# yanqinJiang/Animate3D

Hardware: AMD Instinct MI355X
Metric: UNet denoise-steps/sec, 4view×16frame×512² MV-VDM @1/2/4/8 GPU (higher is better)
Workload: dtype bf16; 1 GPU; BASELINE config 2: 4 views x 16 frames x 512^2 px (64x64 latent), CFG-doubled batch V=8 videos, one MVUNetMotionModel.forward per step, SD1.5 MV-VDM UNet 1.53 B params, seeded synthetic weights; parallelism=single GPU

## Files before the change

animate3d_amd/csrc/gemm_common.h:

```cpp
#pragma once
#include "common.h"

struct GemmParams {
  const uint16_t* X; int64_t ldx;
  const uint16_t* W; int64_t ldw;
  const float* bias;
  const uint16_t* rowbias; int64_t rb_div;
  const uint16_t* R; int64_t ldr;
  uint16_t* Y; int64_t ldy;
  int64_t M, N, K;
  float alpha, beta;
  int vec16;
  int out_f32;
  int B, H, Wd, Cin, Ho, Wo, stride, up, He, We;
  int64_t tiles_n, tiles_m;
  int ksplit, nk_item;
  float* ws; int64_t ws_bytes;
  const uint16_t* X2; int64_t ldx2; int64_t K1;
};

constexpr int EPI_LINEAR = 0, EPI_GEGLU = 1;

static inline int a3d_gemm_kernel_of(int flags) { return flags & A3D_GEMM_KERNEL_MASK; }
static inline int a3d_gemm_reserved_cus_of(int flags) { return flags & A3D_GEMM_RESERVED_CUS_MASK; }
// ... 106 lines not shown
  }
}

template <int NB> A3D_DEV void read_frags(const char* stage, uint32_t xrd, uint32_t wrd, uint32_t wrd_last, uint32_t ko, u32x4_t (&fx)[2],
                                          u32x4_t (&fw)[NB]) {
  const char* xs = stage + xrd;
  const char* ws = stage + wrd;
  const char* wl = stage + wrd_last;
#pragma unroll
  for (int tm = 0; tm < 2; ++tm) fx[tm] = *reinterpret_cast<const u32x4_t*>(xs + tm * 4096 + ko);
#pragma unroll
  for (int tn = 0; tn < NB - 1; ++tn) fw[tn] = *reinterpret_cast<const u32x4_t*>(ws + tn * 4096 + ko);
  fw[NB - 1] = *reinterpret_cast<const u32x4_t*>(wl + ko);
}

template <int EPI, int NB>
A3D_DEV void epilogue_rounded(const GemmParams& p, f32x16_t (&acc)[NB][2], float* const stg, const float* const bias_lds,
                              const uint16_t* const rowbias_lds, const int64_t m0, const int64_t n0, const int wm, const WaveCols<NB> wc,
                              const int lane) {
  const int wblk = wc.first, wblk_last = wc.last;
  auto pass_cols = [&](int ps) { return (2 * ps + 1 < NB) ? 64 : 32; };
  auto pass_col0 = [&](int ps) { return ((2 * ps + 1 < NB) ? wblk + 2 * ps : wblk_last) * 32; };
  const int l31 = lane & 31, g = lane >> 5;
  constexpr int NP = (NB + 1) / 2;
  constexpr int RS = (EPI == EPI_GEGLU) ? 64 : 128;
  char* const stg16 = reinterpret_cast<char*>(stg);
  const int wsw = (EPI == EPI_GEGLU) ? ((l31 >> 1) & 3) : (l31 & 7);
  const int whalf = 8 * (g ^ ((l31 >> 3) & 1));
  auto unswap = [](u32x4_t o, int row) {
    const bool sw = row & 8;
    u32x4_t r;
    r[0] = sw ? o[2] : o[0]; r[1] = sw ? o[3] : o[1]; r[2] = sw ? o[0] : o[2]; r[3] = sw ? o[1] : o[3];
    return r;
  };
// ... 96 lines not shown
      else quads(std::false_type{});
      wave_lds_fence();
      const int lpr = ncol / 8;
      const int cc = lane & (lpr - 1);
      u32x4_t ob[4];
#pragma unroll
      for (int j = 0; j < 4; ++j) {
        if (j * (64 / lpr) >= 32) continue;
        const int row = (64 / lpr) * j + lane / lpr;
        ob[j] = *reinterpret_cast<const u32x4_t*>(sb + row * RS + 16 * (cc ^ (row & 7)));
      }
#pragma unroll
      for (int j = 0; j < 4; ++j) {
        if (j * (64 / lpr) >= 32) continue;
        const int row = (64 / lpr) * j + lane / lpr;
        const int64_t m = mbase + row;
        const u32x4_t o = unswap(ob[j], row);
        *reinterpret_cast<u32x4_t*>(p.Y + m * p.ldy + nbase + 8 * cc) = o;
      }
    }
  }
}

template <int NB>
A3D_DEV void epilogue_residual(const GemmParams& p, f32x16_t (&acc)[NB][2], float* const stg, const float* const bias_lds,
                               const uint16_t* const rowbias_lds, const int64_t m0, const int64_t n0, const int wm, const WaveCols<NB> wc,
                               const int lane) {
  const int l31 = lane & 31, g = lane >> 5;
  constexpr int SROW = 68;
  constexpr int NP = WaveCols<NB>::PASSES;
  u32x4_t rres[2][4];
// ... 78 lines not shown
```

animate3d_amd/csrc/gemm_conv.hip:

```cpp
#include "gemm_common.h"

namespace {

constexpr int BM = 128, BN = 128;
template <int BKT> struct TileCfg {
  static constexpr int LROW = BKT + 8;
  static constexpr int TILE_ELEMS = 128 * LROW;
  static constexpr int STAGE_BYTES = 2 * 2 * TILE_ELEMS * 2;
  static constexpr int EPI_BYTES = 4 * 32 * 68 * 4;
  static constexpr int SMEM_BYTES = STAGE_BYTES > EPI_BYTES ? STAGE_BYTES : EPI_BYTES;
  static constexpr int CPR = BKT / 8;
  static constexpr int RPT = 256 / CPR;
  static constexpr int NPASS = 128 / RPT;
};



template <int CONV, int EPI, int BKT, bool RES>
__global__ __launch_bounds__(256, (BKT == 64 ? 2 : 3)) void gemm_kernel(const GemmParams p) {
  using TC = TileCfg<BKT>;
  constexpr int LROW = TC::LROW, TILE_ELEMS = TC::TILE_ELEMS, NPASS = TC::NPASS, RPT = TC::RPT, BK = BKT;
  extern __shared__ __attribute__((aligned(16))) uint16_t smem[];
  const int tid = threadIdx.x;
  const int lane = tid & 63, wid = tid >> 6;
// ... 537 lines not shown
}

extern "C" int A3D_FN(a3d_conv3x3)(a3d_stream_t stream, const void* X, const void* Wp, const float* bias,
                                const void* rowbias, int64_t rb_div, const void* R, void* Y,
                                int B, int H, int W, int Cin, int Cout, int stride, int up2x, int flags) {
  return conv_entry(stream, X, Wp, bias, rowbias, rb_div, R, Y, B, H, W, Cin, Cout, stride, up2x, flags, nullptr, 0, nullptr);
}

extern "C" int A3D_FN(a3d_conv3x3_ws)(a3d_stream_t stream, const void* X, const void* Wp, const float* bias,
                                   const void* rowbias, int64_t rb_div, const void* R, void* Y,
                                   int B, int H, int W, int Cin, int Cout, int stride, int up2x, int flags,
                                   void* ws, int64_t ws_bytes, int64_t* ws_needed) {
  return conv_entry(stream, X, Wp, bias, rowbias, rb_div, R, Y, B, H, W, Cin, Cout, stride, up2x, flags, ws, ws_bytes, ws_needed);
}

extern "C" int A3D_FN(a3d_gemm_geglu)(a3d_stream_t stream, const void* X, int64_t ldx, const void* W, int64_t ldw,
                                   const float* bias, void* Y, int64_t ldy, int64_t M, int64_t N2, int64_t K, int flags) {
  GemmParams p = dense_params(X, ldx, W, ldw, bias, nullptr, 1, nullptr, 0, Y, ldy, M, N2, K, 1.f, 0.f);
  if (!dense_args_ok(p, 16, 64, 8)) return A3D_EINVAL;
  return launch<0, EPI_GEGLU>((hipStream_t)stream, p, flags);
}
```

animate3d_amd/csrc/gemm_pp.hip:

```cpp
#include "gemm_common.h"

namespace {

constexpr int PBM = 256;
template <int NB> struct PPCfg {
  static constexpr int BN = NB * 64;
  static constexpr int XBYTES = PBM * 128;
  static constexpr int WBYTES = BN * 128;
  static constexpr int EPI_BYTES = 8 * 32 * 68 * 4;
  static constexpr int STAGE = (XBYTES + WBYTES) > EPI_BYTES ? (XBYTES + WBYTES) : EPI_BYTES;
  static constexpr int BIAS_OFF = 2 * STAGE;
  static constexpr int SMEM = BIAS_OFF + 2 * BIAS_IMG_STRIDE;
};

constexpr int PP_GM = 8;
A3D_DEV void pp_tile_coords(int64_t t, int64_t tiles_m, int64_t tiles_n, int64_t& tile_m, int64_t& tile_n) {
  const int64_t gsz = PP_GM * tiles_n;
  const int64_t blk = t / gsz;
  const int64_t first = blk * PP_GM;
  const int64_t gm = tiles_m - first < PP_GM ? tiles_m - first : PP_GM;
  const int64_t within = t - blk * gsz;
  tile_n = within / gm;
  tile_m = first + (within - tile_n * gm);
}

template <int CONV, int EPI, int NB, bool RES, bool SPLIT = false, bool TWO = false>
__global__ __launch_bounds__(512, 1) void gemm_pp_kernel(const GemmParams p) {
  static_assert(!TWO || CONV == 0, "the two-source A operand is a dense-GEMM feature");
  using PC = PPCfg<NB>;
  constexpr int PH = 1, NPH = 4;
  constexpr int NP = 4 + NB;
  extern __shared__ __attribute__((aligned(16))) uint16_t smem[];
  char* const smem_b = reinterpret_cast<char*>(smem);
  const int tid = threadIdx.x, lane = tid & 63;
  const int wid = __builtin_amdgcn_readfirstlane(tid >> 6);
  const int wm = wid >> 1, wn = wid & 1;
  const int grp = wid >> 2;
  const int l31 = lane & 31, g = lane >> 5;
  const int lr = lane >> 3, pos = lane & 7;
  const uint32_t lds0 = lds_addr(smem);

  const int S = SPLIT ? p.ksplit : 1;
  const int64_t ntiles = p.tiles_m * p.tiles_n * S;
  const int64_t G = gridDim.x;
  int64_t t = xcd_remap(blockIdx.x, G);
  if (t >= ntiles) return;
// ... 1 lines not shown

  const uint32_t koff0 = (uint32_t)((g ^ ((l31 >> 1) & 7)) << 4);
  const uint32_t xrd = (uint32_t)(wm * 64 + l31) * 128u;
  const WaveCols<NB> wc(wn);
  const uint32_t wrd = (uint32_t)PC::XBYTES + (uint32_t)(wc.first * 32 + l31) * 128u;
  const uint32_t wrd_last = (uint32_t)PC::XBYTES + (uint32_t)(wc.last * 32 + l31) * 128u;

  const uint32_t vx0 = (uint32_t)(lr * p.ldx * 2 + ((pos ^ (lr >> 1)) << 4));
  const uint32_t vw0 = (uint32_t)(lr * p.ldw * 2 + ((pos ^ (lr >> 1)) << 4));
  uint32_t aoff[CONV ? 4 : 1];
  uint32_t amask[CONV ? 2 : 1];
  uint32_t sok[CONV ? 2 : 1];
  const int64_t cbias = CONV ? ((int64_t)p.Wd + 1) * p.Cin : 0;
  int64_t ld_m0 = 0, ld_n0 = 0;
  int ld_par = 0;
  int ik0 = 0, itap = 0, ikx = 0, iky = 0;
  uint64_t xck = 0;
  uint64_t zpage = 0;
  if constexpr (CONV != 0) {
    zpage = (uint64_t)(uintptr_t)g_zero_page;
    asm volatile("" : "+s"(zpage));
  }
  uint64_t xk = 0, wk = 0, rbk = 0;
  const uint32_t sx8 = (uint32_t)(p.ldx * 16), sw8 = (uint32_t)(p.ldw * 16);
  uint64_t xk2 = 0;
  const uint32_t vx0b = TWO ? (uint32_t)(lr * p.ldx2 * 2 + ((pos ^ (lr >> 1)) << 4)) : 0u;
  const uint32_t sx8b = TWO ? (uint32_t)(p.ldx2 * 16) : 0u;
  auto setup_tile = [&](int64_t tt) {
    int64_t tile_n, tile_m;
    const int64_t tile_id = SPLIT ? (int64_t)((uint32_t)tt / (uint32_t)S) : tt;
    const int64_t kofs = SPLIT ? (CONV ? ((int64_t)(tt - tile_id * S) * nk / 9) * 64 : (int64_t)(tt - tile_id * S) * nk * 64) : 0;
    pp_tile_coords(tile_id, p.tiles_m, p.tiles_n, tile_m, tile_n);
    ld_m0 = tile_m * PBM; ld_n0 = tile_n * PC::BN;
    ik0 = 0; itap = 0; ikx = 0; iky = 0;
    ld_par ^= 1;
    if constexpr (CONV != 0) xck = (uint64_t)(uintptr_t)p.X - (uint64_t)cbias * 2u + (uint64_t)kofs * 2u;
    if constexpr (CONV == 0) xk = (uint64_t)(uintptr_t)(p.X + (ld_m0 + wid * 32) * p.ldx + kofs);
    if constexpr (TWO) xk2 = (uint64_t)(uintptr_t)(p.X2 + (ld_m0 + wid * 32) * p.ldx2);
    wk = (uint64_t)(uintptr_t)(p.W + (ld_n0 + wid * (NB * 8)) * p.ldw + kofs);
    if (EPI == EPI_LINEAR && p.rowbias) rbk = (uint64_t)(uintptr_t)(p.rowbias + (ld_m0 / p.rb_div) * p.N + ld_n0);
    if constexpr (CONV != 0) {
      amask[0] = 0; amask[1] = 0;
#pragma unroll
      for (int i = 0; i < 4; ++i) {
        const int r = (wid * 4 + i) * 8 + lr;
        const int slot = pos ^ ((r >> 1) & 7);
        const uint32_t m = (uint32_t)ld_m0 + (uint32_t)r;
        const uint32_t hw = (uint32_t)(p.Ho * p.Wo);
        const int b = (int)(m / hw);
        const int rem = (int)(m - (uint32_t)b * hw);
        const int oy = (int)((uint32_t)rem / (uint32_t)p.Wo), ox = rem - oy * p.Wo;
        uint32_t mask = 0;
        if constexpr (CONV == 2) {
          const int sy0 = (oy - 1) >> 1, sx0 = (ox - 1) >> 1;
          aoff[i] = (uint32_t)(((((int64_t)b * p.H + sy0) * p.Wd + sx0) * p.Cin + cbias) * 2 + slot * 16);
#pragma unroll
          for (int tp = 0; tp < 9; ++tp) {
            const int yy = oy + tp / 3 - 1, xx = ox + tp % 3 - 1;
            if (yy >= 0 && yy < p.He && xx >= 0 && xx < p.We) mask |= 1u << tp;
          }
          amask[i >> 1] |= (mask << (9 * (i & 1))) | ((uint32_t)(~oy & 1) << (18 + 2 * (i & 1))) | ((uint32_t)(~ox & 1) << (19 + 2 * (i & 1)));
        } else {
          const int y0 = oy * p.stride - 1, x0 = ox * p.stride - 1;
          aoff[i] = (uint32_t)(((((int64_t)b * p.H + y0) * p.Wd + x0) * p.Cin + cbias) * 2 + slot * 16);
#pragma unroll
          for (int tp = 0; tp < 9; ++tp) {
            const int yy = y0 + tp / 3, xx = x0 + tp % 3;
            if (yy >= 0 && yy < p.H && xx >= 0 && xx < p.Wd) mask |= 1u << tp;
          }
          amask[i >> 1] |= mask << (9 * (i & 1));
        }
      }
      sok[0] = 0; sok[1] = 0;
#pragma unroll
      for (int bit = 0; bit < 18; ++bit) {
        if (__builtin_amdgcn_ballot_w64(((amask[0] >> bit) & 1u) != 0u) == ~0ull) sok[0] |= 1u << bit;
        if (__builtin_amdgcn_ballot_w64(((amask[1] >> bit) & 1u) != 0u) == ~0ull) sok[1] |= 1u << bit;
      }
    }
  };
  auto issue_pieces = [&](int buf, auto a_c, auto b_c) __attribute__((always_inline)) {
    constexpr int A = decltype(a_c)::value, B = decltype(b_c)::value;
    if constexpr (A >= B) return;
    const uint32_t dst = lds0 + (uint32_t)buf * PC::STAGE;
    if constexpr (A == 0) {
      if (ik0 == 0) {
        const uint32_t bdst = lds0 + (uint32_t)PC::BIAS_OFF + (uint32_t)ld_par * BIAS_IMG_STRIDE;
        if (p.bias) {
          if (wid == 0) glds16_s((uint32_t)lane * 16u, p.bias + ld_n0, bdst);
          if (NB == 5 && wid == 1) { if (lane < 16) glds16_s((uint32_t)lane * 16u, p.bias + ld_n0 + BIAS_IMG_DMA / 4, bdst + (uint32_t)BIAS_IMG_DMA); }
// ... 3 lines not shown
        }
      }
    }
    if constexpr (CONV != 0) {
      const int ky = iky, kx = ikx;
      const uint32_t rowb = (uint32_t)(p.Wd * p.Cin * 2), colb = (uint32_t)(p.Cin * 2);
      const uint32_t yE = (uint32_t)((ky + 1) >> 1) * rowb, yO = (uint32_t)(ky >> 1) * rowb;
      const uint32_t xE = (uint32_t)((kx + 1) >> 1) * colb, xO = (uint32_t)(kx >> 1) * colb;
#pragma unroll
      for (int i = 0; i < 4; ++i) {
        if (i < A || i >= B) continue;
        const uint32_t d = dst + (uint32_t)(wid * 4 + i) * 1024u;
        const uint32_t mk = amask[i >> 1];
        uint32_t vo = aoff[i];
        if constexpr (CONV == 2) vo += (((mk >> (18 + 2 * (i & 1))) & 1u) ? yE : yO) + (((mk >> (19 + 2 * (i & 1))) & 1u) ? xE : xO);
        const int bit = itap + 9 * (i & 1);
        if ((sok[i >> 1] >> bit) & 1u) {
          glds16_s(vo, (const void*)(uintptr_t)xck, d);
        } else {
          const uint64_t src = ((mk >> bit) & 1u) ? xck + vo : zpage;
          glds16_v((const void*)(uintptr_t)src, d);
        }
      }
    } else {
      const bool sec = TWO && ik0 >= (int)p.K1;
      const uint32_t vxs = sec ? vx0b : vx0, sxs = sec ? sx8b : sx8;
      const uint64_t xks = sec ? xk2 : xk;
#pragma unroll
      for (int i = 0; i < 4; ++i) {
        if (i < A || i >= B) continue;
        const int pc = wid * 4 + i;
        glds16_s(vxs ^ (uint32_t)((i & 1) << 6), (const void*)(uintptr_t)(xks + (uint64_t)(uint32_t)(i * sxs)), dst + (uint32_t)pc * 1024u);
      }
    }
#pragma unroll
    for (int i = 0; i < NB; ++i) {
      if (4 + i < A || 4 + i >= B) continue;
      const int pc = wid * NB + i;
      glds16_s(vw0 ^ (uint32_t)((pc & 1) << 6), (const void*)(uintptr_t)(wk + (uint64_t)(uint32_t)(i * sw8)), dst + (uint32_t)PC::XBYTES + (uint32_t)pc * 1024u);
    }
    if constexpr (B == NP) {
      if constexpr (CONV != 0) {
        const uint64_t cin2 = (uint64_t)(uint32_t)p.Cin * 2u;
        wk += cin2;
        ++itap;
        if (++ikx == 3) { ikx = 0; ++iky; }
        if (itap == 9) {
          itap = 0; iky = 0; wk -= 9u * cin2 - 128u;
          if constexpr (CONV == 1) xck -= (2u * (uint64_t)(uint32_t)p.Wd + 2u) * cin2;
          xck += 128u;
        } else if constexpr (CONV == 1) {
          xck += ikx == 0 ? ((uint64_t)(uint32_t)p.Wd - 2u) * cin2 : cin2;
        }
      } else {
        if (TWO && ik0 >= (int)p.K1) xk2 += 128; else xk += 128;
        wk += 128;
      }
      ik0 += 64;
    }
  };
  auto issue_phase = [&](int buf, auto ph_c, bool late) __attribute__((always_inline)) {
    constexpr int ph = decltype(ph_c)::value;
    using I0 = std::integral_constant<int, 0>;
    using I3 = std::integral_constant<int, 3>;
    using I5 = std::integral_constant<int, 5>;
    using I6 = std::integral_constant<int, 6>;
    using IN = std::integral_constant<int, NP>;
// ... 19 lines not shown
#pragma unroll
      for (int tn = 0; tn < NB; ++tn)
#pragma unroll
        for (int tm = 0; tm < 2; ++tm) acc[tn][tm] = mfma32(fw[s][tn], fx[s][tm], acc[tn][tm]);
  };

  zero_absent_bias_images<512>(smem_b + PC::BIAS_OFF, p.bias, EPI == EPI_LINEAR ? p.rowbias : nullptr, tid);
  setup_tile(t);
  issue_pieces(0, std::integral_constant<int, 0>{}, std::integral_constant<int, NP>{});
  asm volatile("s_waitcnt vmcnt(0)" ::: "memory");
  tile_barrier();
  int buf = 0;
  for (;;) {
    int64_t tile_n, tile_m;
    pp_tile_coords(SPLIT ? (int64_t)((uint32_t)t / (uint32_t)S) : t, p.tiles_m, p.tiles_n, tile_m, tile_n);
    const int64_t m0 = tile_m * PBM, n0 = tile_n * PC::BN;
    const int64_t tnext = t + G;
#pragma unroll
    for (int a = 0; a < NB; ++a)
#pragma unroll
      for (int b = 0; b < 2; ++b)
#pragma unroll
        for (int r = 0; r < 16; ++r) acc[a][b][r] = 0.f;
    const int cur_par = ld_par;
    if (grp) tile_barrier();
    for (int kt = 0; kt < nk; ++kt) {
      const bool last = kt + 1 >= nk;
      const bool more = !last || tnext < ntiles;
      const bool late = kt == 0;
      static_for<NPH>([&](auto ph_c) __attribute__((always_inline)) {
        constexpr int ph = decltype(ph_c)::value;
// ... 20 lines not shown

    if constexpr (SPLIT) {
      float* const wsi = p.ws + ((t * 8 + wid) * (NB * 8)) * 256 + lane * 4;
#pragma unroll
      for (int tn = 0; tn < NB; ++tn)
#pragma unroll
        for (int tm = 0; tm < 2; ++tm)
#pragma unroll
          for (int q = 0; q < 4; ++q)
            *reinterpret_cast<float4*>(wsi + ((tn * 2 + tm) * 4 + q) * 256) =
                float4{acc[tn][tm][4 * q], acc[tn][tm][4 * q + 1], acc[tn][tm][4 * q + 2], acc[tn][tm][4 * q + 3]};
    } else {
      float* const stg = reinterpret_cast<float*>(smem_b + (buf ^ 1) * PC::STAGE) + wid * (32 * 68);
      const float* const bias_lds = bias_image(smem_b + PC::BIAS_OFF, cur_par);
      const uint16_t* const rowbias_lds = rowbias_image(smem_b + PC::BIAS_OFF, cur_par);
      if constexpr (EPI == EPI_GEGLU || !RES) epilogue_rounded<EPI, NB>(p, acc, stg, bias_lds, rowbias_lds, m0, n0, wm, wc, lane);
      else epilogue_residual<NB>(p, acc, stg, bias_lds, rowbias_lds, m0, n0, wm, wc, lane);
    }
    if (tnext >= ntiles) break;
    t = tnext;
  }
}

template <int NB>
__global__ __launch_bounds__(512) void splitk_reduce_kernel(const GemmParams p) {
  using PC = PPCfg<NB>;
  const int tid = threadIdx.x, lane = tid & 63, wid = tid >> 6;
  const int wm = wid >> 1, wn = wid & 1, l31 = lane & 31, g = lane >> 5;
  const WaveCols<NB> wc(wn);
  const int S = p.ksplit;
  int64_t tile_n, tile_m;
// ... 74 lines not shown
  if (p.ksplit > 1) {
    if (nb == 5) return launch_pp<CONV, EPI_LINEAR, 5, false, true>(stream, p, cus);
    if (nb == 4) return launch_pp<CONV, EPI_LINEAR, 4, false, true>(stream, p, cus);
    return A3D_EUNSUPPORTED;
  }
  if (nb == 5) return p.R ? launch_pp<CONV, EPI_LINEAR, 5, true>(stream, p, cus) : launch_pp<CONV, EPI_LINEAR, 5, false>(stream, p, cus);
  if (nb == 4) return p.R ? launch_pp<CONV, EPI_LINEAR, 4, true>(stream, p, cus) : launch_pp<CONV, EPI_LINEAR, 4, false>(stream, p, cus);
  return A3D_EUNSUPPORTED;
}

}

int A3D_FN(a3d_launch_gemm_pp)(int conv, int epi, int nb, hipStream_t stream, const GemmParams& p, int cus) {
  if (conv == 0) return launch_pp_conv<0>(epi, nb, stream, p, cus);
  if (conv == 1) return launch_pp_conv<1>(epi, nb, stream, p, cus);
  return launch_pp_conv<2>(epi, nb, stream, p, cus);
}
```

animate3d_amd/hip_ops.py:

```python
from __future__ import annotations

import ctypes
import os
import re
from dataclasses import dataclass
from typing import NamedTuple, Optional

import torch

_PKG = os.path.dirname(os.path.abspath(__file__))
_LIB_PATH = os.path.join(_PKG, "lib", "libanimate3d_hip.so")
_HEADER_PATH = os.path.join(os.path.dirname(_PKG), "include", "animate3d_hip.h")
_lib = None

c_i64, c_int, c_f32, c_f64, c_vp = ctypes.c_int64, ctypes.c_int, ctypes.c_float, ctypes.c_double, ctypes.c_void_p


class _RowMapC(ctypes.Structure):
    _fields_ = [("gdiv", c_i64), ("ga", c_i64), ("gb", c_i64), ("seg_len", c_i64), ("seg_stride", c_i64), ("ld", c_i64)]


class StageAdamEntry(ctypes.Structure):
    _fields_ = [("p", c_vp), ("g", c_vp), ("m", c_vp), ("v", c_vp), ("step", c_vp), ("n", c_i64), ("lr", c_f64)]

# ... 84 lines not shown


def rowmap_rows(m: RowMap, groups: int, step: int, length: int, device="cpu") -> torch.Tensor:
    g = torch.arange(0, groups, step, device=device).view(-1, 1)
    s = torch.arange(length, device=device).view(1, -1)
    return ((g // m.gdiv) * m.ga + (g % m.gdiv) * m.gb + (s // m.seg_len) * m.seg_stride + s % m.seg_len).reshape(-1)


def rowmap_covers(m: RowMap, groups: int, step: int, length: int, rows: int, device="cpu") -> bool:
    if (groups + step - 1) // step * length != rows:
        return False
    idx = rowmap_rows(m, groups, step, length, device)
    return bool(int(idx.min()) >= 0 and int(idx.max()) < rows and torch.unique(idx).numel() == rows)


def lib_path() -> str:
    return _LIB_PATH


def load_library():
    global _lib
    if _lib is None:
        if not os.path.exists(_LIB_PATH):
            raise RuntimeError(f"{_LIB_PATH} is missing: run `python -m animate3d_amd.build` (or __graft_entry__.build()). "
                               "There is no CPU fallback for the MI355X kernels.")
        functions = read_header(_HEADER_PATH).functions
        lib = ctypes.CDLL(_LIB_PATH)
        for name, (res, args) in functions.items():
            fn = getattr(lib, name)
            fn.restype, fn.argtypes = res, args
# ... 42 lines not shown
        return method(self, *args, **kwargs)
    return wrapper


class _Entry:

    def __init__(self, lib, f16: bool):
        for name in EXPORTED_SYMBOLS:
            twin = (name[:-5] if name.endswith("_bf16") else name) + "_f16"
            setattr(self, name, getattr(lib, twin if f16 and twin in EXPORTED_SYMBOLS else name))


class HipOps:

    has_attn_lse = True

    def __init__(self, device: Optional[torch.device] = None, act_dtype: torch.dtype = torch.bfloat16, split_k: bool = True):
        if not torch.cuda.is_available():
            raise RuntimeError("HipOps needs a visible MI355X (torch.cuda.is_available() is False); no CPU fallback exists")
        if act_dtype not in (torch.bfloat16, torch.float16):
            raise ValueError(f"storage type {act_dtype} is not supported (bfloat16 or float16)")
        self.raw_lib = load_library()
        self._kv_row_cache = {}
        self._kv_cover_cache = {}
        self.act_dtype = act_dtype
        self.lib = _Entry(self.raw_lib, act_dtype == torch.float16)
        self.device = torch.device(device) if device is not None else torch.device("cuda", torch.cuda.current_device())
        self.reserved_cus = 0
        self.split_k = bool(split_k)
        self.split_k_gemm = False
# ... 94 lines not shown
        n = w.shape[0] // 2
        assert n % 32 == 0
        h, g = w[:n].reshape(n // 32, 32, *w.shape[1:]), w[n:].reshape(n // 32, 32, *w.shape[1:])
        return torch.stack([h, g], dim=1).reshape(w.shape).contiguous()

    def gemm_geglu(self, x, w_il, bias_il, *, tile128: bool = False):
        x, w_il = self._act(x, "geglu.x"), self._act(w_il, "geglu.w")
        M, K = x.shape
        N2 = w_il.shape[0]
        y = self.empty(M, N2 // 2)
        self._launch("a3d_gemm_geglu_bf16", _p(x), x.stride(0), _p(w_il), w_il.stride(0), _p(bias_il), _p(y), y.stride(0), M, N2, K,
                     self._gemm_flags(tile128), what=f"M={M} N2={N2} K={K}")
        return y

    def conv3x3(self, x, B: int, H: int, W: int, w, bias, *, stride: int = 1, up2x: bool = False, rowbias=None, rb_div: int = 1, residual=None,
                up_size=None, tile128: bool = False):
        x, w = self._act(x, "conv.x"), self._act(w, "conv.w")
        Cin = x.shape[1]
        Cout = w.shape[0]
        assert x.is_contiguous() and w.is_contiguous() and x.shape[0] == B * H * W and w.shape[1] == 9 * Cin
        He, We = (2 * H, 2 * W) if up2x else (H, W)
        up_code = 1 if up2x else 0
        if up_size is not None:
            if not up2x or up_size[0] not in (2 * H, 2 * H - 1) or up_size[1] not in (2 * W, 2 * W - 1):
                raise ValueError(f"forced upsample size {tuple(up_size)} is not reachable from {(H, W)} (2x or 2x - 1 per axis)")
            He, We = int(up_size[0]), int(up_size[1])
            up_code |= (2 if He == 2 * H - 1 else 0) | (4 if We == 2 * W - 1 else 0)
        Ho, Wo = (He - 1) // stride + 1, (We - 1) // stride + 1
        y = self.empty(B * Ho * Wo, Cout)
        if residual is not None:
            assert residual.is_contiguous() and residual.shape == y.shape
        if rowbias is not None:
            assert rowbias.is_contiguous() and rowbias.shape[1] == Cout
        flags = self._gemm_flags(tile128)
        args = (_p(x), _p(w), _p(bias), _p(rowbias), rb_div, _p(residual), _p(y), B, H, W, Cin, Cout, stride, up_code, flags)
# ... 399 lines not shown
```

animate3d_amd/unet.py:

```python
from __future__ import annotations

import math
import os
import re
from types import SimpleNamespace
from typing import Any, Dict, Optional, Tuple, Union

import torch
import torch.nn as nn

from . import modules as M
from .config import UNetConfig
from .embeddings import sine_pos_2d, sinusoidal_pos_1d
from .hip_ops import RowMap, on_model_device


class UNet3DConditionOutput:

    def __init__(self, sample: torch.Tensor):
        self.sample = sample

    def __getitem__(self, i):
        return (self.sample,)[i]


def _rows(w: torch.Tensor, r0: int, r1: Optional[int] = None) -> torch.Tensor:
    r1 = w.shape[0] if r1 is None else r1
    if getattr(w, "_a3d_sink", None) is None:
        return w[r0:r1]
# ... 2 lines not shown


class MVUNetMotionModel(nn.Module):
    def __init__(self, config: Optional[UNetConfig] = None, ops=None, num_views: Optional[int] = None,
                 device: Optional[Union[str, torch.device]] = None, **config_overrides):
        super().__init__()
        cfg = config if config is not None else UNetConfig(**config_overrides)
        self.config = cfg
        self.sample_size = cfg.sample_size
        self.num_views = num_views
        self._ops = ops
        self._ops_auto = False
        self._packed = None
        self._packed_frozen = None
        self._pack_grad = False
        self._train_ops = None
        self._active_ops = None
        self._cond = None
        self.stack_conditioning = True
        self._pe_cache: Dict[Tuple[int, int, int], torch.Tensor] = {}
        self.parallel = None
        self._frames = (0, 0)
        if len(cfg.block_out_channels) != len(cfg.down_has_attn):
            raise ValueError("block_out_channels and down_has_attn must have the same length")
        if 9 * cfg.in_channels > 64:
            raise ValueError(f"in_channels = {cfg.in_channels} is not supported (<= 7; the MV-VDM UNet has 4 — the 9-channel PIA conv_in "
                             "of unet_motion_mv_model.py:312-330 is not on this path)")
        ctx = torch.device(device) if device is not None else torch.device("cpu")
        with ctx:
            self._build(cfg)
# ... 402 lines not shown
                    parts.append((ci, pr.to_out_i2v))
                bias = None
                for c, lin in parts:
                    if lin.bias is not None:
                        bias = float(c) * lin.bias.detach().float() if bias is None else bias + float(c) * lin.bias.detach().float()
                ns.om = (self._w(torch.cat([float(c) * lin.weight.detach().float() for c, lin in parts], dim=1)), self._f(bias))
            attns.append(ns)
        out = SimpleNamespace(norm=(self._f(m.norm.weight), self._f(m.norm.bias)),
                              pin=(self._w(m.proj_in.weight), self._f(m.proj_in.bias)),
                              attns=attns,
                              pout=(self._w(m.proj_out.weight), self._f(m.proj_out.bias)))
        out.ff = self._pack_ff(tb)
        return out

    def _pack_block(self, blk: M.MotionBlock):
        return SimpleNamespace(
            resnets=[self._pack_resnet(r) for r in blk.resnets],
            t2d=[self._pack_t2d(t) for t in blk.attentions] if blk.has_cross_attention else None,
            motion=[self._pack_motion(m) for m in blk.motion_modules],
            down=None if blk.downsamplers is None else (self._conv_w(blk.downsamplers[0].conv), self._f(blk.downsamplers[0].conv.bias)),
            up=None if blk.upsamplers is None else (self._conv_w(blk.upsamplers[0].conv), self._f(blk.upsamplers[0].conv.bias)))

    def _pack(self):
        cfg = self.config
        dev = self.device
        te, P = self.time_embedding, SimpleNamespace()
        P.time = (self._w(te.linear_1.weight), self._f(te.linear_1.bias), self._w(te.linear_2.weight), self._f(te.linear_2.bias))
        P.cam = None
        if cfg.camera_embedding_dim is not None:
            ce = self.camera_embedding
            w1 = torch.zeros(ce.linear_1.weight.shape[0], 64, device=dev, dtype=torch.float32)
            w1[:, : cfg.camera_embedding_dim] = ce.linear_1.weight.detach().float()
            P.cam = (self._w(w1), self._f(ce.linear_1.bias), self._w(ce.linear_2.weight), self._f(ce.linear_2.bias))
        P.ip = None
        if self.encoder_hid_proj is not None:
            ipl = self.encoder_hid_proj.image_projection_layers[0]
# ... 372 lines not shown
        self._gradient_checkpointing = False

    def _mark_persistent(self, node):
        if torch.is_tensor(node):
            node._a3d_persistent = True
        elif isinstance(node, SimpleNamespace):
            for v in vars(node).values():
                self._mark_persistent(v)
        elif isinstance(node, (list, tuple)):
            for v in node:
                self._mark_persistent(v)

    def _pack_train(self):
        sig = tuple(p.requires_grad for p in self.parameters())
        if self._packed_frozen is None or sig != getattr(self, "_packed_frozen_sig", None):
            self._packed_frozen = self._pack()
            self._packed_frozen_sig = sig
            self._packed = None
            self._mark_persistent(self._packed_frozen)
            if getattr(self, "_train_ops", None) is not None:
                self._train_ops._persistent.clear()
        Pf = self._packed_frozen
        trainable = lambda m: m is not None and any(p.requires_grad for p in m.parameters())
        for name, mod in (("time_embedding", self.time_embedding), ("camera_embedding", getattr(self, "camera_embedding", None)),
                          ("encoder_hid_proj", self.encoder_hid_proj), ("conv_in", self.conv_in), ("conv_norm_out", self.conv_norm_out),
                          ("conv_out", self.conv_out)):
            if trainable(mod):
                raise NotImplementedError(f"{name} is not trainable on this path (the reference trains 'motion_modules.' and 'i2v.' only)")
        self._pack_grad = True
        self._coef_tensors = []
        try:
# ... 207 lines not shown
        pk = P.mid
        x = layer(x, pk.resnets[0], pk.t2d[0], pk.motion[0], h_, w_)
        x = self._resnet(x, B2, h_, w_, pk.resnets[1], semb, rb_rows)
        if mid_block_additional_residual is not None:
            x = plus(x, mid_block_additional_residual, h_, w_)
        lvl = len(sizes) - 1
        for bi, (blk, pk) in enumerate(zip(self.up_blocks, P.up)):
            for j, rp in enumerate(pk.resnets):
                skip = skips.pop()
                if getattr(self, "_freeu_factors", None) is not None:
                    x, skip = self._freeu(bi, x, skip, B2, h_, w_)
                pair = self._active_ops is None and hasattr(ops, "gemm2") and hasattr(ops, "group_norm2")
                x = layer((x, skip) if pair else ops.concat(x, skip), rp, pk.t2d[j] if pk.t2d is not None else None, pk.motion[j], h_, w_)
            if pk.up is not None:
                lvl -= 1
                x, h_, w_ = ops.conv3x3(x, B2, h_, w_, pk.up[0], pk.up[1], up2x=True, up_size=sizes[lvl])
        x = ops.group_norm(x, B2, h_ * w_, P.norm_out[0], P.norm_out[1], cfg.norm_num_groups, cfg.norm_eps, True)
        x, _, _ = ops.conv3x3(x, B2, h_, w_, P.conv_out[0], P.conv_out[1])
        out_dtype = sample.dtype if sample.dtype in (torch.float32, torch.bfloat16, torch.float16) else torch.float32
        out = ops.unpack_out(x, V, cfg.out_channels, F, H, W, out_dtype)
        if par is not None:
            out = par.all_gather_output(out, V_full, n_full, F_full)
        if not return_dict:
            return (out,)
        return UNet3DConditionOutput(sample=out)
```

animate3d_amd/vae.py:

```python
from __future__ import annotations

from dataclasses import dataclass
from types import SimpleNamespace
from typing import Optional, Tuple, Union

import torch
import torch.nn as nn

from .autograd_ops import AutogradOps
from .denoise import randn_like_reference
from .hip_ops import on_model_device


@dataclass
class VAEConfig:
    block_out_channels: Tuple[int, ...] = (128, 256, 512, 512)
    layers_per_block: int = 2
    norm_num_groups: int = 32
    latent_channels: int = 4
    out_channels: int = 3
    scaling_factor: float = 0.18215
    attention_head_dim: int = 512


class _Resnet(nn.Module):
    def __init__(self, cin, cout, groups):
# ... 204 lines not shown
        P = SimpleNamespace()
        P.pq = (self.post_quant_conv.weight.detach().float().reshape(cfg.latent_channels, cfg.latent_channels).contiguous(),
                self._f(self.post_quant_conv.bias))
        wi = d.conv_in.weight.detach().float().permute(0, 2, 3, 1).reshape(d.conv_in.weight.shape[0], -1)
        wpad = wi.new_zeros(wi.shape[0], 64)
        wpad[:, : wi.shape[1]] = wi
        P.conv_in = (self._w(wpad), self._f(d.conv_in.bias))
        a = d.mid_block.attentions[0]
        P.mid = SimpleNamespace(
            r0=self._pack_resnet(d.mid_block.resnets[0]), r1=self._pack_resnet(d.mid_block.resnets[1]),
            gn=(self._f(a.group_norm.weight), self._f(a.group_norm.bias)),
            q=(self._w(a.to_q.weight), self._f(a.to_q.bias)), k=(self._w(a.to_k.weight), self._f(a.to_k.bias)),
            v=(self._w(a.to_v.weight), self._f(a.to_v.bias)), o=(self._w(a.to_out[0].weight), self._f(a.to_out[0].bias)))
        P.up = [SimpleNamespace(res=[self._pack_resnet(r) for r in b.resnets],
                                up=None if b.upsamplers is None else self._conv_w(b.upsamplers[0].conv)) for b in d.up_blocks]
        P.norm_out = (self._f(d.conv_norm_out.weight), self._f(d.conv_norm_out.bias))
        P.conv_out = self._conv_w(d.conv_out, pad_out_to=4)
        self._packed = P
        return P

    def _decode_rows(self, z: torch.Tensor, scale: float):
        ops, cfg = self.ops, self.config
        P = self._packed if self._packed is not None else self._pack()
        B, Cz, H, W = z.shape
        z = ops.channel_mix(z.to(device=self.device, dtype=torch.float32).contiguous(), P.pq[0], P.pq[1], scale)
        x = ops.gemm(ops.im2col_in(z.reshape(B, Cz, 1, H, W)), P.conv_in[0], P.conv_in[1])
        x = self._resnet(x, B, H, W, P.mid.r0)
        x = self._mid_attention(x, B, H, W, P.mid)
        x = self._resnet(x, B, H, W, P.mid.r1)
        for blk in P.up:
            for r in blk.res:
                x = self._resnet(x, B, H, W, r)
            if blk.up is not None:
                x, H, W = ops.conv3x3(x, B, H, W, blk.up[0], blk.up[1], up2x=True)
        x = ops.group_norm(x, B, H * W, P.norm_out[0], P.norm_out[1], cfg.norm_num_groups, 1e-6, True)
        x, _, _ = ops.conv3x3(x, B, H, W, P.conv_out[0], P.conv_out[1])
        return x, H, W

    @torch.no_grad()
    @on_model_device
    def decode(self, z: torch.Tensor, scale: float = 1.0) -> torch.Tensor:
        x, H, W = self._decode_rows(z, scale)
        img = self.ops.unpack_out(x, z.shape[0], 4, 1, H, W, torch.float32)
        return img[:, : self.config.out_channels, 0].contiguous()

    @torch.no_grad()
    def decode_latents(self, latents: torch.Tensor) -> torch.Tensor:
        b, c, f, h, w = latents.shape
        z = latents.permute(0, 2, 1, 3, 4).reshape(b * f, c, h, w)
# ... 134 lines not shown
```

include/animate3d_hip.h:

```cpp
#ifndef ANIMATE3D_HIP_H
#define ANIMATE3D_HIP_H

#include <stdint.h>

#ifdef __cplusplus
extern "C" {
#endif

typedef void* a3d_stream_t;

enum {
  A3D_OK = 0,
  A3D_EINVAL = -1,
  A3D_EUNSUPPORTED = -2
};

enum { A3D_F32 = 0, A3D_BF16 = 1, A3D_F16 = 2 };

const char* a3d_version(void);

typedef struct a3d_rowmap {
  int64_t gdiv, ga, gb;
  int64_t seg_len, seg_stride;
  int64_t ld;
// ... 17 lines not shown

int a3d_gemm_f32out_bf16(a3d_stream_t stream, const void* X, int64_t ldx, const void* W, int64_t ldw,
                         const float* bias, float* Y, int64_t ldy, int64_t M, int64_t N, int64_t K, float alpha);

int a3d_gemm_geglu_bf16(a3d_stream_t stream, const void* X, int64_t ldx, const void* W, int64_t ldw,
                        const float* bias, void* Y, int64_t ldy, int64_t M, int64_t N2, int64_t K, int flags);

int a3d_conv3x3_bf16(a3d_stream_t stream, const void* X, const void* Wp, const float* bias,
                     const void* rowbias, int64_t rb_div, const void* R, void* Y,
                     int B, int H, int W, int Cin, int Cout, int stride, int up2x, int flags);

int a3d_conv3x3_ws_bf16(a3d_stream_t stream, const void* X, const void* Wp, const float* bias,
                        const void* rowbias, int64_t rb_div, const void* R, void* Y,
                        int B, int H, int W, int Cin, int Cout, int stride, int up2x, int flags,
                        void* ws, int64_t ws_bytes, int64_t* ws_needed);

#define A3D_ATTN_ACCUMULATE 1
#define A3D_ATTN_CAUSAL 2
#define A3D_ATTN_EXACT 4
#define A3D_ATTN_PLAIN 8
int a3d_flash_attn_bf16(a3d_stream_t stream, const void* Q, const void* K, const void* V, void* O,
                        const a3d_rowmap* qmap, const a3d_rowmap* kmap, const a3d_rowmap* omap,
                        int groups, int heads, int head_dim, int64_t q_len, int64_t kv_len,
                        float scale, float out_scale, int accumulate);

int a3d_flash_attn_counted_bf16(a3d_stream_t stream, const void* Q, const void* K, const void* V, void* O,
                                const a3d_rowmap* qmap, const a3d_rowmap* kmap, const a3d_rowmap* omap,
                                int groups, int heads, int head_dim, int64_t q_len, int64_t kv_len,
                                float scale, float out_scale, int accumulate, unsigned int* counters);

// ... 247 lines not shown
                    void* Y, int64_t ldy, int64_t M, int64_t N, int64_t K, float alpha, float beta, int flags,
                    void* ws, int64_t ws_bytes, int64_t* ws_needed);
int a3d_gemm2_f16(a3d_stream_t stream, const void* X, int64_t ldx, const void* X2, int64_t ldx2, int64_t K1,
                  const void* W, int64_t ldw, const float* bias, void* Y, int64_t ldy, int64_t M, int64_t N, int64_t K, int flags);
int a3d_gemm_f32out_f16(a3d_stream_t stream, const void* X, int64_t ldx, const void* W, int64_t ldw,
                         const float* bias, float* Y, int64_t ldy, int64_t M, int64_t N, int64_t K, float alpha);
int a3d_gemm_geglu_f16(a3d_stream_t stream, const void* X, int64_t ldx, const void* W, int64_t ldw,
                        const float* bias, void* Y, int64_t ldy, int64_t M, int64_t N2, int64_t K, int flags);
int a3d_conv3x3_f16(a3d_stream_t stream, const void* X, const void* Wp, const float* bias,
                     const void* rowbias, int64_t rb_div, const void* R, void* Y,
                     int B, int H, int W, int Cin, int Cout, int stride, int up2x, int flags);
int a3d_conv3x3_ws_f16(a3d_stream_t stream, const void* X, const void* Wp, const float* bias,
                       const void* rowbias, int64_t rb_div, const void* R, void* Y,
                       int B, int H, int W, int Cin, int Cout, int stride, int up2x, int flags,
                       void* ws, int64_t ws_bytes, int64_t* ws_needed);
int a3d_flash_attn_f16(a3d_stream_t stream, const void* Q, const void* K, const void* V, void* O,
                        const a3d_rowmap* qmap, const a3d_rowmap* kmap, const a3d_rowmap* omap,
                        int groups, int heads, int head_dim, int64_t q_len, int64_t kv_len,
                        float scale, float out_scale, int accumulate);
int a3d_flash_attn_counted_f16(a3d_stream_t stream, const void* Q, const void* K, const void* V, void* O,
                               const a3d_rowmap* qmap, const a3d_rowmap* kmap, const a3d_rowmap* omap,
                               int groups, int heads, int head_dim, int64_t q_len, int64_t kv_len,
                               float scale, float out_scale, int accumulate, unsigned int* counters);
int a3d_flash_attn2_f16(a3d_stream_t stream, const void* Q, const void* K, const void* V, const void* K2, const void* V2, void* O,
                        const a3d_rowmap* qmap, const a3d_rowmap* kmap, const a3d_rowmap* kmap2, const a3d_rowmap* omap,
                        int groups, int heads, int head_dim, int64_t q_len, int64_t kv_len, int64_t kv_len2,
                        float scale, float out_scale, float out_scale2, int accumulate);
int a3d_temporal_attn_f16(a3d_stream_t stream, const void* Q, const void* K, const void* V, int64_t ldqkv,
                           void* O, int64_t ldo, int videos, int frames, int64_t L, int heads,
                           int head_dim, float scale);
// ... 68 lines not shown
```

Before: 2.400 denoise-steps/s.

## Fold nearest-upsample into 3x3 conv as four 2x2 phase convolutions

Replaces the up2x-then-3x3 convolution in the UNet and VAE upsamplers with four phase-specific 2x2 convolutions over the source-resolution input. Weights are pre-summed per output phase at pack time in float64, then rounded once to the activation dtype. A new CONV==3 mode in the persistent GEMM kernel selects the phase from the tile index and scatters output rows through an up-sampling row map. K shrinks from 9*Cin to 4*Cin per output pixel, cutting upsampler FLOPs by more than half. The trade-off is a different rounding order, extra folded-weight memory, and a path that only runs when the shape and alignment conditions hold (no residual or rowbias, not training).

```diff
diff --git a/animate3d_amd/csrc/gemm_common.h b/animate3d_amd/csrc/gemm_common.h
--- a/animate3d_amd/csrc/gemm_common.h
+++ b/animate3d_amd/csrc/gemm_common.h
@@ -144,10 +144,11 @@
   fw[NB - 1] = *reinterpret_cast<const u32x4_t*>(wl + ko);
 }
 
-template <int EPI, int NB>
+template <int EPI, int NB, bool UPROW = false>
 A3D_DEV void epilogue_rounded(const GemmParams& p, f32x16_t (&acc)[NB][2], float* const stg, const float* const bias_lds,
                               const uint16_t* const rowbias_lds, const int64_t m0, const int64_t n0, const int wm, const WaveCols<NB> wc,
-                              const int lane) {
+                              const int lane, const uint32_t uprow = 0) {
+  static_assert(!UPROW || EPI == EPI_LINEAR, "the up-sampling row map is a feature of the linear epilogue");
   const int wblk = wc.first, wblk_last = wc.last;
   auto pass_cols = [&](int ps) { return (2 * ps + 1 < NB) ? 64 : 32; };
   auto pass_col0 = [&](int ps) { return ((2 * ps + 1 < NB) ? wblk + 2 * ps : wblk_last) * 32; };
@@ -274,7 +275,11 @@
       for (int j = 0; j < 4; ++j) {
         if (j * (64 / lpr) >= 32) continue;
         const int row = (64 / lpr) * j + lane / lpr;
-        const int64_t m = mbase + row;
+        int64_t m = mbase + row;
+        if constexpr (UPROW) {
+          const uint32_t ms = (uint32_t)m;
+          m = (int64_t)(4u * ms - 2u * (ms % (uint32_t)p.Wd) + uprow);
+        }
         const u32x4_t o = unswap(ob[j], row);
         *reinterpret_cast<u32x4_t*>(p.Y + m * p.ldy + nbase + 8 * cc) = o;
       }
diff --git a/animate3d_amd/csrc/gemm_conv.hip b/animate3d_amd/csrc/gemm_conv.hip
--- a/animate3d_amd/csrc/gemm_conv.hip
+++ b/animate3d_amd/csrc/gemm_conv.hip
@@ -575,6 +575,42 @@
   return conv_entry(stream, X, Wp, bias, rowbias, rb_div, R, Y, B, H, W, Cin, Cout, stride, up2x, flags, ws, ws_bytes, ws_needed);
 }
 
+extern "C" int A3D_FN(a3d_conv3x3_up2x_folded)(a3d_stream_t stream, const void* X, const void* Wf, const float* bias,
+                                            const void* rowbias, const void* R, void* Y,
+                                            int B, int H, int W, int Cin, int Cout, int flags) {
+  if (!X || !Wf || !Y || B <= 0 || H <= 0 || W <= 0 || Cin <= 0 || Cout <= 0) return A3D_EINVAL;
+  if (rowbias || R) return A3D_EINVAL;
+  if (!gemm_flags_ok(flags) || a3d_gemm_kernel_of(flags) != 0) return A3D_EINVAL;
+  if (Cin % 64 != 0 || (Cout % 320 != 0 && Cout % 256 != 0)) return A3D_EINVAL;
+  const int64_t msrc = (int64_t)B * H * W;
+  if (msrc % PBM != 0) return A3D_EINVAL;
+  if (!a3d_aligned(16, X, Wf) || !a3d_aligned(16, bias) || !a3d_aligned(16, Y)) return A3D_EINVAL;
+  if (((uint64_t)msrc + 2u * (uint64_t)W + 2u) * (uint64_t)Cin * 2u >= (1ull << 32) || (uint64_t)Cin * 64u >= (1ull << 31)) return A3D_EINVAL;
+  const int cus_dev = device_cus();
+  if (cus_dev == 0) return A3D_EUNSUPPORTED;
+  const int reserved = a3d_gemm_reserved_cus_of(flags);
+  GemmParams p{};
+  p.X = (const uint16_t*)X; p.ldx = Cin; p.W = (const uint16_t*)Wf; p.ldw = (int64_t)4 * Cin;
+  p.bias = bias; p.rb_div = 1; p.Y = (uint16_t*)Y; p.ldy = Cout; p.ldr = Cout;
+  p.B = B; p.H = H; p.Wd = W; p.Cin = Cin; p.stride = 1; p.up = 1; p.He = 2 * H; p.We = 2 * W;
+  p.Ho = H; p.Wo = W;
+  p.M = 4 * msrc; p.N = Cout; p.K = (int64_t)4 * Cin;
+  p.alpha = 1.f; p.beta = 1.f; p.vec16 = 1;
+  p.ksplit = 1; p.nk_item = (int)(p.K / 64);
+  p.tiles_m = p.M / PBM;
+  int nb = 0;
+  int64_t best = -1;
+  for (int cand = 5; cand >= 4; --cand) {
+    if (Cout % (cand * 64) != 0) continue;
+    const int64_t tiles = p.tiles_m * (Cout / (cand * 64));
+    const int64_t rounds = (tiles + cus_dev - 1) / cus_dev;
+    const int64_t cost = rounds * (p.nk_item + 12) * cand * (cand == 4 ? 108 : 100);
+    if (best < 0 || cost < best) { best = cost; nb = cand; }
+  }
+  p.tiles_n = Cout / (nb * 64);
+  return A3D_FN(a3d_launch_gemm_pp)(3, EPI_LINEAR, nb, (hipStream_t)stream, p, cus_dev - reserved > 32 ? cus_dev - reserved : 32);
+}
+
 extern "C" int A3D_FN(a3d_gemm_geglu)(a3d_stream_t stream, const void* X, int64_t ldx, const void* W, int64_t ldw,
                                    const float* bias, void* Y, int64_t ldy, int64_t M, int64_t N2, int64_t K, int flags) {
   GemmParams p = dense_params(X, ldx, W, ldw, bias, nullptr, 1, nullptr, 0, Y, ldy, M, N2, K, 1.f, 0.f);
diff --git a/animate3d_amd/csrc/gemm_pp.hip b/animate3d_amd/csrc/gemm_pp.hip
--- a/animate3d_amd/csrc/gemm_pp.hip
+++ b/animate3d_amd/csrc/gemm_pp.hip
@@ -30,6 +30,8 @@
   using PC = PPCfg<NB>;
   constexpr int PH = 1, NPH = 4;
   constexpr int NP = 4 + NB;
+  constexpr int TW = CONV == 3 ? 2 : 3;
+  constexpr int NT = TW * TW;
   extern __shared__ __attribute__((aligned(16))) uint16_t smem[];
   char* const smem_b = reinterpret_cast<char*>(smem);
   const int tid = threadIdx.x, lane = tid & 63;
@@ -61,6 +63,7 @@
   const int64_t cbias = CONV ? ((int64_t)p.Wd + 1) * p.Cin : 0;
   int64_t ld_m0 = 0, ld_n0 = 0;
   int ld_par = 0;
+  int ld_ph = 0;
   int ik0 = 0, itap = 0, ikx = 0, iky = 0;
   uint64_t xck = 0;
   uint64_t zpage = 0;
@@ -79,12 +82,17 @@
     const int64_t kofs = SPLIT ? (CONV ? ((int64_t)(tt - tile_id * S) * nk / 9) * 64 : (int64_t)(tt - tile_id * S) * nk * 64) : 0;
     pp_tile_coords(tile_id, p.tiles_m, p.tiles_n, tile_m, tile_n);
     ld_m0 = tile_m * PBM; ld_n0 = tile_n * PC::BN;
+    if constexpr (CONV == 3) {
+      const uint32_t tsrc = (uint32_t)p.tiles_m >> 2;
+      ld_ph = (int)((uint32_t)tile_m / tsrc);
+      ld_m0 = (int64_t)((uint32_t)tile_m - (uint32_t)ld_ph * tsrc) * PBM;
+    }
     ik0 = 0; itap = 0; ikx = 0; iky = 0;
     ld_par ^= 1;
     if constexpr (CONV != 0) xck = (uint64_t)(uintptr_t)p.X - (uint64_t)cbias * 2u + (uint64_t)kofs * 2u;
     if constexpr (CONV == 0) xk = (uint64_t)(uintptr_t)(p.X + (ld_m0 + wid * 32) * p.ldx + kofs);
     if constexpr (TWO) xk2 = (uint64_t)(uintptr_t)(p.X2 + (ld_m0 + wid * 32) * p.ldx2);
-    wk = (uint64_t)(uintptr_t)(p.W + (ld_n0 + wid * (NB * 8)) * p.ldw + kofs);
+    wk = (uint64_t)(uintptr_t)(p.W + ((CONV == 3 ? (int64_t)ld_ph * p.N : 0) + ld_n0 + wid * (NB * 8)) * p.ldw + kofs);
     if (EPI == EPI_LINEAR && p.rowbias) rbk = (uint64_t)(uintptr_t)(p.rowbias + (ld_m0 / p.rb_div) * p.N + ld_n0);
     if constexpr (CONV != 0) {
       amask[0] = 0; amask[1] = 0;
@@ -108,19 +116,19 @@
           }
           amask[i >> 1] |= (mask << (9 * (i & 1))) | ((uint32_t)(~oy & 1) << (18 + 2 * (i & 1))) | ((uint32_t)(~ox & 1) << (19 + 2 * (i & 1)));
         } else {
-          const int y0 = oy * p.stride - 1, x0 = ox * p.stride - 1;
+          const int y0 = oy * p.stride - 1 + (CONV == 3 ? ld_ph >> 1 : 0), x0 = ox * p.stride - 1 + (CONV == 3 ? ld_ph & 1 : 0);
           aoff[i] = (uint32_t)(((((int64_t)b * p.H + y0) * p.Wd + x0) * p.Cin + cbias) * 2 + slot * 16);
 #pragma unroll
-          for (int tp = 0; tp < 9; ++tp) {
-            const int yy = y0 + tp / 3, xx = x0 + tp % 3;
+          for (int tp = 0; tp < NT; ++tp) {
+            const int yy = y0 + tp / TW, xx = x0 + tp % TW;
             if (yy >= 0 && yy < p.H && xx >= 0 && xx < p.Wd) mask |= 1u << tp;
           }
-          amask[i >> 1] |= mask << (9 * (i & 1));
+          amask[i >> 1] |= mask << (NT * (i & 1));
         }
       }
       sok[0] = 0; sok[1] = 0;
 #pragma unroll
-      for (int bit = 0; bit < 18; ++bit) {
+      for (int bit = 0; bit < 2 * NT; ++bit) {
         if (__builtin_amdgcn_ballot_w64(((amask[0] >> bit) & 1u) != 0u) == ~0ull) sok[0] |= 1u << bit;
         if (__builtin_amdgcn_ballot_w64(((amask[1] >> bit) & 1u) != 0u) == ~0ull) sok[1] |= 1u << bit;
       }
@@ -154,7 +162,7 @@
         const uint32_t mk = amask[i >> 1];
         uint32_t vo = aoff[i];
         if constexpr (CONV == 2) vo += (((mk >> (18 + 2 * (i & 1))) & 1u) ? yE : yO) + (((mk >> (19 + 2 * (i & 1))) & 1u) ? xE : xO);
-        const int bit = itap + 9 * (i & 1);
+        const int bit = itap + NT * (i & 1);
         if ((sok[i >> 1] >> bit) & 1u) {
           glds16_s(vo, (const void*)(uintptr_t)xck, d);
         } else {
@@ -184,13 +192,13 @@
         const uint64_t cin2 = (uint64_t)(uint32_t)p.Cin * 2u;
         wk += cin2;
         ++itap;
-        if (++ikx == 3) { ikx = 0; ++iky; }
-        if (itap == 9) {
-          itap = 0; iky = 0; wk -= 9u * cin2 - 128u;
-          if constexpr (CONV == 1) xck -= (2u * (uint64_t)(uint32_t)p.Wd + 2u) * cin2;
+        if (++ikx == TW) { ikx = 0; ++iky; }
+        if (itap == NT) {
+          itap = 0; iky = 0; wk -= (uint64_t)NT * cin2 - 128u;
+          if constexpr (CONV != 2) xck -= ((uint64_t)(TW - 1) * (uint64_t)(uint32_t)p.Wd + (uint64_t)(TW - 1)) * cin2;
           xck += 128u;
-        } else if constexpr (CONV == 1) {
-          xck += ikx == 0 ? ((uint64_t)(uint32_t)p.Wd - 2u) * cin2 : cin2;
+        } else if constexpr (CONV != 2) {
+          xck += ikx == 0 ? ((uint64_t)(uint32_t)p.Wd - (uint64_t)(TW - 1)) * cin2 : cin2;
         }
       } else {
         if (TWO && ik0 >= (int)p.K1) xk2 += 128; else xk += 128;
@@ -240,7 +248,15 @@
   for (;;) {
     int64_t tile_n, tile_m;
     pp_tile_coords(SPLIT ? (int64_t)((uint32_t)t / (uint32_t)S) : t, p.tiles_m, p.tiles_n, tile_m, tile_n);
-    const int64_t m0 = tile_m * PBM, n0 = tile_n * PC::BN;
+    int64_t m0 = tile_m * PBM;
+    const int64_t n0 = tile_n * PC::BN;
+    uint32_t uprow = 0;
+    if constexpr (CONV == 3) {
+      const uint32_t tsrc = (uint32_t)p.tiles_m >> 2;
+      const uint32_t ph = (uint32_t)tile_m / tsrc;
+      m0 = (int64_t)((uint32_t)tile_m - ph * tsrc) * PBM;
+      uprow = (ph >> 1) * 2u * (uint32_t)p.Wd + (ph & 1u);
+    }
     const int64_t tnext = t + G;
 #pragma unroll
     for (int a = 0; a < NB; ++a)
@@ -291,7 +307,7 @@
       float* const stg = reinterpret_cast<float*>(smem_b + (buf ^ 1) * PC::STAGE) + wid * (32 * 68);
       const float* const bias_lds = bias_image(smem_b + PC::BIAS_OFF, cur_par);
       const uint16_t* const rowbias_lds = rowbias_image(smem_b + PC::BIAS_OFF, cur_par);
-      if constexpr (EPI == EPI_GEGLU || !RES) epilogue_rounded<EPI, NB>(p, acc, stg, bias_lds, rowbias_lds, m0, n0, wm, wc, lane);
+      if constexpr (EPI == EPI_GEGLU || !RES) epilogue_rounded<EPI, NB, CONV == 3>(p, acc, stg, bias_lds, rowbias_lds, m0, n0, wm, wc, lane, uprow);
       else epilogue_residual<NB>(p, acc, stg, bias_lds, rowbias_lds, m0, n0, wm, wc, lane);
     }
     if (tnext >= ntiles) break;
@@ -396,5 +412,9 @@
 int A3D_FN(a3d_launch_gemm_pp)(int conv, int epi, int nb, hipStream_t stream, const GemmParams& p, int cus) {
   if (conv == 0) return launch_pp_conv<0>(epi, nb, stream, p, cus);
   if (conv == 1) return launch_pp_conv<1>(epi, nb, stream, p, cus);
-  return launch_pp_conv<2>(epi, nb, stream, p, cus);
-}
+  if (conv == 2) return launch_pp_conv<2>(epi, nb, stream, p, cus);
+  if (conv != 3 || epi != EPI_LINEAR || p.R || p.rowbias || p.ksplit > 1 || p.X2) return A3D_EUNSUPPORTED;
+  if (nb == 5) return launch_pp<3, EPI_LINEAR, 5, false>(stream, p, cus);
+  if (nb == 4) return launch_pp<3, EPI_LINEAR, 4, false>(stream, p, cus);
+  return A3D_EUNSUPPORTED;
+}
diff --git a/animate3d_amd/hip_ops.py b/animate3d_amd/hip_ops.py
--- a/animate3d_amd/hip_ops.py
+++ b/animate3d_amd/hip_ops.py
@@ -122,6 +122,49 @@
     return bool(int(idx.min()) >= 0 and int(idx.max()) < rows and torch.unique(idx).numel() == rows)
 
 
+UP2X_TAPS = (((0,), (1, 2)), ((0, 1), (2,)))
+
+
+def fold_up2x_sums(w: torch.Tensor) -> torch.Tensor:
+    Cout, K9 = w.shape
+    if K9 % 9:
+        raise ValueError(f"a packed 3x3 weight has 9 Cin columns, got {tuple(w.shape)}")
+    w64 = w.detach().to(device="cpu", dtype=torch.float64).view(Cout, 3, 3, K9 // 9)
+    wf = torch.zeros((4, Cout, 2, 2, K9 // 9), dtype=torch.float64)
+    for a in range(2):
+        for b in range(2):
+            for r in range(2):
+                for c in range(2):
+                    for ky in UP2X_TAPS[a][r]:
+                        for kx in UP2X_TAPS[b][c]:
+                            wf[2 * a + b, :, r, c] += w64[:, ky, kx]
+    return wf.view(4, Cout, 4 * (K9 // 9))
+
+
+def round_once(x64: torch.Tensor, dtype: torch.dtype) -> torch.Tensor:
+    f = x64.to(torch.float32)
+    inexact = f.to(torch.float64) != x64
+    over = f.to(torch.float64).abs() > x64.abs()
+    f = torch.where(over, torch.nextafter(f, torch.zeros_like(f)), f)
+    bits = f.view(torch.int32) | inexact.to(torch.int32)
+    return bits.view(torch.float32).to(dtype)
+
+
+def fold_up2x_weights(w: torch.Tensor, dtype: Optional[torch.dtype] = None) -> torch.Tensor:
+    return round_once(fold_up2x_sums(w), dtype or w.dtype).to(w.device).contiguous()
+
+
+def up2x_folded_applies(B: int, H: int, W: int, Cin: int, Cout: int, *, up2x: bool, up_size=None, stride: int = 1, rowbias=None,
+                        residual=None, folded=None, tile128: bool = False, shape_independent: bool = False) -> bool:
+    if folded is None or not up2x or stride != 1 or rowbias is not None or residual is not None or tile128 or shape_independent:
+        return False
+    if up_size is not None and (int(up_size[0]), int(up_size[1])) != (2 * H, 2 * W):
+        return False
+    if (B * H * W) % 256 or Cin % 64 or (Cout % 320 and Cout % 256):
+        return False
+    return (B * H * W + 2 * W + 2) * Cin * 2 < 1 << 32
+
+
 def lib_path() -> str:
     return _LIB_PATH
 
@@ -194,6 +237,7 @@
 class HipOps:
 
     has_attn_lse = True
+    has_up2x_folded = True
 
     def __init__(self, device: Optional[torch.device] = None, act_dtype: torch.dtype = torch.bfloat16, split_k: bool = True):
         if not torch.cuda.is_available():
@@ -318,11 +362,20 @@
         return y
 
     def conv3x3(self, x, B: int, H: int, W: int, w, bias, *, stride: int = 1, up2x: bool = False, rowbias=None, rb_div: int = 1, residual=None,
-                up_size=None, tile128: bool = False):
+                up_size=None, tile128: bool = False, folded=None):
         x, w = self._act(x, "conv.x"), self._act(w, "conv.w")
         Cin = x.shape[1]
         Cout = w.shape[0]
         assert x.is_contiguous() and w.is_contiguous() and x.shape[0] == B * H * W and w.shape[1] == 9 * Cin
+        if up2x_folded_applies(B, H, W, Cin, Cout, up2x=up2x, up_size=up_size, stride=stride, rowbias=rowbias, residual=residual,
+                               folded=folded, tile128=tile128, shape_independent=not self.split_k):
+            assert folded.dtype == self.act_dtype and folded.is_cuda and folded.is_contiguous() and folded.shape == (4, Cout, 4 * Cin)
+            if bias is not None:
+                assert bias.dtype == torch.float32 and bias.numel() == Cout
+            y = self.empty(4 * B * H * W, Cout)
+            self._launch("a3d_conv3x3_up2x_folded_bf16", _p(x), _p(folded), _p(bias), None, None, _p(y), B, H, W, Cin, Cout,
+                         self._gemm_flags(False), what=f"B={B} H={H} W={W} Cin={Cin} Cout={Cout}")
+            return y, 2 * H, 2 * W
         He, We = (2 * H, 2 * W) if up2x else (H, W)
         up_code = 1 if up2x else 0
         if up_size is not None:
diff --git a/animate3d_amd/unet.py b/animate3d_amd/unet.py
--- a/animate3d_amd/unet.py
+++ b/animate3d_amd/unet.py
@@ -12,7 +12,7 @@
 from . import modules as M
 from .config import UNetConfig
 from .embeddings import sine_pos_2d, sinusoidal_pos_1d
-from .hip_ops import RowMap, on_model_device
+from .hip_ops import RowMap, fold_up2x_weights, on_model_device
 
 
 class UNet3DConditionOutput:
@@ -45,6 +45,7 @@
         self._packed = None
         self._packed_frozen = None
         self._pack_grad = False
+        self._pack_fold = True
         self._train_ops = None
         self._active_ops = None
         self._cond = None
@@ -477,12 +478,15 @@
         return out
 
     def _pack_block(self, blk: M.MotionBlock):
+        up = None if blk.upsamplers is None else (self._conv_w(blk.upsamplers[0].conv), self._f(blk.upsamplers[0].conv.bias))
+        fold = up is not None and self._pack_fold and not self._pack_grad and getattr(self.ops, "has_up2x_folded", False)
         return SimpleNamespace(
+            up_folded=fold_up2x_weights(up[0]) if fold else None,
             resnets=[self._pack_resnet(r) for r in blk.resnets],
             t2d=[self._pack_t2d(t) for t in blk.attentions] if blk.has_cross_attention else None,
             motion=[self._pack_motion(m) for m in blk.motion_modules],
             down=None if blk.downsamplers is None else (self._conv_w(blk.downsamplers[0].conv), self._f(blk.downsamplers[0].conv.bias)),
-            up=None if blk.upsamplers is None else (self._conv_w(blk.upsamplers[0].conv), self._f(blk.upsamplers[0].conv.bias)))
+            up=up)
 
     def _pack(self):
         cfg = self.config
@@ -885,7 +889,11 @@
     def _pack_train(self):
         sig = tuple(p.requires_grad for p in self.parameters())
         if self._packed_frozen is None or sig != getattr(self, "_packed_frozen_sig", None):
-            self._packed_frozen = self._pack()
+            self._pack_fold = False
+            try:
+                self._packed_frozen = self._pack()
+            finally:
+                self._pack_fold = True
             self._packed_frozen_sig = sig
             self._packed = None
             self._mark_persistent(self._packed_frozen)
@@ -1123,7 +1131,8 @@
                 x = layer((x, skip) if pair else ops.concat(x, skip), rp, pk.t2d[j] if pk.t2d is not None else None, pk.motion[j], h_, w_)
             if pk.up is not None:
                 lvl -= 1
-                x, h_, w_ = ops.conv3x3(x, B2, h_, w_, pk.up[0], pk.up[1], up2x=True, up_size=sizes[lvl])
+                fold = {"folded": pk.up_folded} if self._active_ops is None and getattr(pk, "up_folded", None) is not None else {}
+                x, h_, w_ = ops.conv3x3(x, B2, h_, w_, pk.up[0], pk.up[1], up2x=True, up_size=sizes[lvl], **fold)
         x = ops.group_norm(x, B2, h_ * w_, P.norm_out[0], P.norm_out[1], cfg.norm_num_groups, cfg.norm_eps, True)
         x, _, _ = ops.conv3x3(x, B2, h_, w_, P.conv_out[0], P.conv_out[1])
         out_dtype = sample.dtype if sample.dtype in (torch.float32, torch.bfloat16, torch.float16) else torch.float32
diff --git a/animate3d_amd/vae.py b/animate3d_amd/vae.py
--- a/animate3d_amd/vae.py
+++ b/animate3d_amd/vae.py
@@ -9,7 +9,7 @@
 
 from .autograd_ops import AutogradOps
 from .denoise import randn_like_reference
-from .hip_ops import on_model_device
+from .hip_ops import fold_up2x_weights, on_model_device
 
 
 @dataclass
@@ -244,6 +244,8 @@
             v=(self._w(a.to_v.weight), self._f(a.to_v.bias)), o=(self._w(a.to_out[0].weight), self._f(a.to_out[0].bias)))
         P.up = [SimpleNamespace(res=[self._pack_resnet(r) for r in b.resnets],
                                 up=None if b.upsamplers is None else self._conv_w(b.upsamplers[0].conv)) for b in d.up_blocks]
+        for blk in P.up:
+            blk.up_folded = fold_up2x_weights(blk.up[0]) if blk.up is not None and getattr(self.ops, "has_up2x_folded", False) else None
         P.norm_out = (self._f(d.conv_norm_out.weight), self._f(d.conv_norm_out.bias))
         P.conv_out = self._conv_w(d.conv_out, pad_out_to=4)
         self._packed = P
@@ -262,7 +264,8 @@
             for r in blk.res:
                 x = self._resnet(x, B, H, W, r)
             if blk.up is not None:
-                x, H, W = ops.conv3x3(x, B, H, W, blk.up[0], blk.up[1], up2x=True)
+                fold = {"folded": blk.up_folded} if blk.up_folded is not None else {}
+                x, H, W = ops.conv3x3(x, B, H, W, blk.up[0], blk.up[1], up2x=True, **fold)
         x = ops.group_norm(x, B, H * W, P.norm_out[0], P.norm_out[1], cfg.norm_num_groups, 1e-6, True)
         x, _, _ = ops.conv3x3(x, B, H, W, P.conv_out[0], P.conv_out[1])
         return x, H, W
diff --git a/include/animate3d_hip.h b/include/animate3d_hip.h
--- a/include/animate3d_hip.h
+++ b/include/animate3d_hip.h
@@ -55,6 +55,10 @@
                         const void* rowbias, int64_t rb_div, const void* R, void* Y,
                         int B, int H, int W, int Cin, int Cout, int stride, int up2x, int flags,
                         void* ws, int64_t ws_bytes, int64_t* ws_needed);
+
+int a3d_conv3x3_up2x_folded_bf16(a3d_stream_t stream, const void* X, const void* Wf, const float* bias,
+                                 const void* rowbias, const void* R, void* Y,
+                                 int B, int H, int W, int Cin, int Cout, int flags);
 
 #define A3D_ATTN_ACCUMULATE 1
 #define A3D_ATTN_CAUSAL 2
@@ -332,6 +336,9 @@
                        const void* rowbias, int64_t rb_div, const void* R, void* Y,
                        int B, int H, int W, int Cin, int Cout, int stride, int up2x, int flags,
                        void* ws, int64_t ws_bytes, int64_t* ws_needed);
+int a3d_conv3x3_up2x_folded_f16(a3d_stream_t stream, const void* X, const void* Wf, const float* bias,
+                                const void* rowbias, const void* R, void* Y,
+                                int B, int H, int W, int Cin, int Cout, int flags);
 int a3d_flash_attn_f16(a3d_stream_t stream, const void* Q, const void* K, const void* V, void* O,
                         const a3d_rowmap* qmap, const a3d_rowmap* kmap, const a3d_rowmap* omap,
                         int groups, int heads, int head_dim, int64_t q_len, int64_t kv_len,
```

After: 2.430 denoise-steps/s (median of 6 runs). 1.01x the previous value.
